# gk969/stm32-speech-recognition

Measured on AMD Instinct MI355X. Metric: utterances/sec (256-frame, 100 templates), higher is better.
Workload: dtype int32

## Files before the change

### stm32_speech_recognition_amd/csrc/k_mfcc.hip

```cpp
#include "sr_fft_dev.h"

#include <type_traits>

#ifndef SR_MEL_CHUNKED
#define SR_MEL_CHUNKED 1
#endif

namespace sr {

constexpr int kMfccWaves = 4;
constexpr int kFramesPerWave = 16, kFramesPerWaveMid = 4, kFramesPerWaveSmall = 1;
#ifndef SR_MAG_TAB_BINS
#define SR_MAG_TAB_BINS 8
#endif
constexpr int mfcc_tab_bins(int fpw) { return fpw == kFramesPerWave ? SR_MAG_TAB_BINS : 0; }
static_assert(SR_MAG_TAB_BINS == 0 || SR_MAG_TAB_BINS == 4 || SR_MAG_TAB_BINS == 8, "table bins per lane");
#ifndef SR_MFCC_PIPE
#define SR_MFCC_PIPE 1
#endif
#ifndef SR_MFCC_PIPE_PEEL
#define SR_MFCC_PIPE_PEEL 1
#endif
#ifndef SR_MFCC_PIPE_VMCNT
#define SR_MFCC_PIPE_VMCNT (SR_MFCC_PIPE_PEEL ? 3 : 0)
#endif
static_assert(SR_MFCC_PIPE_VMCNT == 0 || (SR_MFCC_PIPE_VMCNT == 3 && SR_MFCC_PIPE_PEEL), "younger loads counted by the wait");
constexpr bool mfcc_pipelined(int fpw) { return SR_MFCC_PIPE && mfcc_tab_bins(fpw) == 8; }
constexpr int kMelPad = kMel + 1;
__device__ __forceinline__ constexpr int mel_chunk_word(int j) { return 256 * ((j >> 2) & 1) + 4 * ((j >> 3) ^ (4 * ((j >> 2) & 1))) + (j & 3); }
constexpr int mfcc_wave_lds_words(int fpw) { return kXchgWords + fpw * kMelPad + 64; }

template <typename Base>
struct MfccTabArgs : Base {
    const uint16_t *mag_q;
    uint32_t mag_table_off;
};
template <typename Base>
constexpr int mfcc_feat_kind<MfccTabArgs<Base>> = mfcc_feat_kind<Base>;
template <typename Base>
static MfccTabArgs<Base> mfcc_tab_args(const Base &b, const MfccMagTab &tab)
{
    MfccTabArgs<Base> r;
    static_cast<Base &>(r) = b;
    r.mag_q = tab.mag_q;
    r.mag_table_off = tab.mag_table_off;
    return r;
}

template <int kFPW, typename Args = MfccTabArgs<MfccArgs>>
__global__ void __launch_bounds__(64 * kMfccWaves, 4) k_mfcc(const Args a)
{
    constexpr int kFeat = mfcc_feat_kind<Args>;
    constexpr uint32_t kFeatW = (kFeat == SR_FEAT_FFT || kFeat == SR_FEAT_MAG) ? kBins : kMel;
    constexpr int kWaveLdsWords = mfcc_wave_lds_words(kFPW);
    constexpr int kTabBins = mfcc_tab_bins(kFPW);
    constexpr bool kPipe = mfcc_pipelined(kFPW);
    extern __shared__ __attribute__((aligned(16))) uint32_t smem[];
    __shared__ uint32_t s_dctM[kCoef * kMelPad];
    __shared__ int s_dctS[kCoef * kMelPad];
    __shared__ u32x4 s_tw3[kTw3Row * 4], s_tw5[8 * 64];
    __shared__ u32x4 s_tm[4 * 64];
    const int lane = threadIdx.x & 63, w = __builtin_amdgcn_readfirstlane(threadIdx.x >> 6);
    uint32_t *buf = smem + w * kWaveLdsWords;
    uint32_t *xw = buf;
    uint32_t *powb = buf + kXchgWords, *moff = powb + kFPW * kMelPad;

    for (int i = threadIdx.x; i < kCoef * kMel; i += blockDim.x) {
        const int c = a.t.dct[i], o = (i / kMel) * kMelPad + i % kMel;
        s_dctM[o] = (uint32_t)(((c < 0 ? -c : c) * 262144 + 99) / 100);
        s_dctS[o] = (c > 0) - (c < 0);
    }
    __syncthreads();

    LaneTw tw;
    load_lane_tw(a.t, lane, tw);
    if (w == 0 && lane < 4) {
        const uint32_t *f = &tw.s3[0][0][0];
#pragma unroll
        for (int c = 0; c < 8; c++) s_tw3[lane * kTw3Row + c] = u32x4{f[4 * c], f[4 * c + 1], f[4 * c + 2], f[4 * c + 3]};
    }
    if (w == 1 % kMfccWaves) store_tw32(s_tw5, lane, tw.s5);
#ifndef SR_INJECT_LDS_RACE
    if (w == 2 % kMfccWaves) {
#pragma unroll
        for (int c = 0; c < 2; c++) {
            s_tm[64 * c + lane] = *(const u32x4 *)(a.t.tri_even_m + 8 * lane + 4 * c);
            s_tm[64 * (c + 2) + lane] = *(const u32x4 *)(a.t.tri_odd_m + 8 * lane + 4 * c);
        }
    }
#endif
    __syncthreads();
#ifdef SR_INJECT_LDS_RACE
    if (w == 2 % kMfccWaves) {
#if SR_INJECT_LDS_RACE >= 2
        __builtin_amdgcn_s_sleep(127);
#endif
#pragma unroll
        for (int c = 0; c < 2; c++) {
            s_tm[64 * c + lane] = *(const u32x4 *)(a.t.tri_even_m + 8 * lane + 4 * c);
            s_tm[64 * (c + 2) + lane] = *(const u32x4 *)(a.t.tri_odd_m + 8 * lane + 4 * c);
        }
    }
#endif
    int hamm_m[3];
#pragma unroll
    for (int k = 0; k < 3; k++) hamm_m[k] = (lane + 64 * k < kFrameLen) ? hamm_fused_multiplier(a.t.hamm[lane + 64 * k]) : 0;
    int f_lo = 0, p_hi = 0, p_lo = 0, x_hi = 0, x_lo = 0;
    if (lane < kMel) {
        const int h = lane;
        f_lo = (h == 0) ? 0 : (int)a.t.tri_cen[h - 1];
        const int f_hi = (h == kMel - 1) ? kBins : (int)a.t.tri_cen[h + 1];
        const int ih = f_hi - 1, il = f_lo ? f_lo - 1 : 0, half = (h & 1) ? kBins : 0;
#if SR_MEL_CHUNKED
        p_hi = half + mel_chunk_word(ih), x_hi = (ih >> 3) > 0 ? (ih >> 3) - 1 : 0;
        p_lo = half + mel_chunk_word(il), x_lo = (il >> 3) > 0 ? (il >> 3) - 1 : 0;
#else
        p_hi = half + ih, x_hi = (ih >> 3) > 0 ? (ih >> 3) - 1 : 0;
        p_lo = half + il, x_lo = (il >> 3) > 0 ? (il >> 3) - 1 : 0;
#endif
    }
    const uint64_t mag_p = (uint64_t)a.mag_q;
    const u32x4 mag_rs = {(uint32_t)mag_p, (uint32_t)(mag_p >> 32) | (2u << 16), kMagTabEntries, 0x00027000u};
    const uint32_t tw_off = 32u * (uint32_t)lane;
#if SR_MEL_CHUNKED
    const int e_base = mel_chunk_word(lane);
    constexpr int kEs = 32, kEh = 128;
    const int c0 = mel_chunk_word(8 * lane), c1 = mel_chunk_word(8 * lane + 4);
#else
    const int e_base = lane;
    constexpr int kEs = 64, kEh = 256;
    const int c0 = 8 * lane, c1 = 8 * lane + 4;
#endif

    uint32_t item = blockIdx.x;
    uint32_t nx_nfrm = 0;
    int nx_mid = 0, nx_seg0 = 0;
    if (item < a.n_items) {
        const sr_vad_rec *rec = a.vad + item / a.tiles;
        nx_nfrm = rec->frm_num;
        nx_mid = (int)rec->atap.mid_val;
        nx_seg0 = rec->seg[0];
    }
    for (; item < a.n_items; item += gridDim.x) {
        const uint32_t b = item / a.tiles, tile = item - b * a.tiles;
        const uint32_t nfrm = nx_nfrm;
        const int mid = nx_mid, seg0 = nx_seg0;
        if (item + gridDim.x < a.n_items) {
            const sr_vad_rec *rec = a.vad + (item + gridDim.x) / a.tiles;
            nx_nfrm = rec->frm_num;
            nx_mid = (int)rec->atap.mid_val;
            nx_seg0 = rec->seg[0];
        }
        const uint16_t *row = a.pcm + (uint64_t)b * a.pcm_stride;
        int16_t *out = a.mfcc + (uint64_t)b * a.max_frames * kCoef;
        const uint32_t f0 = tile * (kMfccWaves * kFPW) + w * kFPW;
        uint32_t *frow = nullptr;
        if constexpr (kFeat != 0) frow = a.feat + (uint64_t)b * a.max_frames * kFeatW;
        uint32_t nf = 0;
        if (f0 < nfrm) nf = (nfrm - f0 < (uint32_t)kFPW) ? nfrm - f0 : (uint32_t)kFPW;

        uint32_t s_pp[3] = {0, 0, 0};
        if (nf) {
            const uint16_t *x = row + seg0 + (int)kHop * (int)f0;
#pragma unroll
            for (int k = 0; k < 3; k++) {
                const int i = lane + 64 * k;
                if (i < kFrameLen) s_pp[k] = *(const u32_align2 *)(x + i - 1);
            }
        }
        if constexpr (!kPipe)
        for (uint32_t fi = 0; fi < nf; fi++) {
#pragma unroll
            for (int k = 0; k < 3; k++) {
                const int i = lane + 64 * k;
                if (i < kFrameLen) xw[i] = k == 0 ? window_sample<4>(s_pp[k], mid, hamm_m[k]) : window_sample<2>(s_pp[k], mid, hamm_m[k]);
            }
            if (fi + 1 < nf) {
                const uint16_t *x = row + seg0 + (int)kHop * (int)(f0 + fi + 1);
#pragma unroll
                for (int k = 0; k < 3; k++) {
                    const int i = lane + 64 * k;
                    if (i < kFrameLen) s_pp[k] = *(const u32_align2 *)(x + i - 1);
                }
            }
            wave_sync();
            uint32_t v[4][4], u[4][4];
            fft_front_real160(xw, lane, tw, s_tw3, v);
            fft_exchange(buf, lane, v, u);
#pragma unroll
            for (int e4 = 0; e4 < 4; e4++)
                bfly_pk<false>(u[0][e4], u[1][e4], u[2][e4], u[3][e4], tw.s4[0][0], tw.s4[0][1], tw.s4[1][0], tw.s4[1][1],
                               tw.s4[2][0], tw.s4[2][1], tw.s4[3][0], tw.s4[3][1]);
            wave_sync();
            uint32_t k5[4][4][2];
            load_tw32(s_tw5, lane, k5);
            uint32_t nn[8];
#pragma unroll
            for (int e3 = 0; e3 < 4; e3++) {
                bfly_pk<true>(u[e3][0], u[e3][1], u[e3][2], u[e3][3], k5[e3][0][0], k5[e3][0][1], k5[e3][1][0],
                              k5[e3][1][1], k5[e3][2][0], k5[e3][2][1], k5[e3][3][0], k5[e3][3][1]);
                if constexpr (kFeat == SR_FEAT_FFT) {
                    uint32_t *fr = frow + (f0 + fi) * kFeatW + lane + 64 * e3;
                    fr[0] = u[e3][0];
                    fr[256] = u[e3][1];
                }
                nn[2 * e3] = (uint32_t)sdot2z(u[e3][0], u[e3][0]);
                nn[2 * e3 + 1] = (uint32_t)sdot2z(u[e3][1], u[e3][1]);
            }
            const uint32_t nmax = max(max(max(max(nn[0], nn[1]), nn[2]), max(max(nn[3], nn[4]), nn[5])), max(nn[6], nn[7]));
#ifdef SR_TESTING
            const bool quiet = __builtin_expect(__builtin_amdgcn_ballot_w64(nmax > kMagSmallMax) == 0 && !a.mag_table_off, 1);
#else
            const bool quiet = __builtin_expect(__builtin_amdgcn_ballot_w64(nmax > kMagSmallMax) == 0, 1);
#endif
            u32x4 tw_e[2], tw_o[2];
            bool cheap = true;
            if (!quiet) {
#pragma unroll
                for (int c = 0; c < 2; c++) {
                    tw_e[c] = *(const u32x4 *)((const char *)a.t.tri_even32 + tw_off + 16 * c);
                    tw_o[c] = *(const u32x4 *)((const char *)a.t.tri_odd32 + tw_off + 16 * c);
                }
                cheap = __builtin_amdgcn_ballot_w64(nmax > a.mag_cheap_max) == 0;
            } else {
                asm volatile("" : "=v"(tw_e[0]), "=v"(tw_e[1]), "=v"(tw_o[0]), "=v"(tw_o[1]));
            }
            uint32_t *eb = buf + e_base;
            if (kTabBins > 0 && quiet) {
                uint32_t tq[8];
#pragma unroll
                for (int e3 = 0; e3 < 4; e3++) {
                    if constexpr (kTabBins == 8)
                        asm volatile("buffer_load_ushort %0, %1, %2, 0 idxen" : "=v"(tq[2 * e3]) : "v"(nn[2 * e3]), "s"(mag_rs));
                    asm volatile("buffer_load_ushort %0, %1, %2, 0 idxen" : "=v"(tq[2 * e3 + 1]) : "v"(nn[2 * e3 + 1]), "s"(mag_rs));
                }
                uint32_t q0s[4];
                if constexpr (kTabBins == 4) {
#pragma unroll
                    for (int e3 = 0; e3 < 4; e3++) q0s[e3] = cvt_u32(__builtin_amdgcn_sqrtf((float)(int)nn[2 * e3]) * 10.0f) << 2;
                }
                if constexpr (kTabBins == 8)
                    asm volatile("s_waitcnt vmcnt(0)" : "+v"(tq[0]), "+v"(tq[1]), "+v"(tq[2]), "+v"(tq[3]), "+v"(tq[4]), "+v"(tq[5]), "+v"(tq[6]), "+v"(tq[7]));
                else
                    asm volatile("s_waitcnt vmcnt(0)" : "+v"(tq[1]), "+v"(tq[3]), "+v"(tq[5]), "+v"(tq[7]));
#pragma unroll
                for (int e3 = 0; e3 < 4; e3++) {
                    uint32_t q0, q1 = tq[2 * e3 + 1];
                    if constexpr (kTabBins == 8) q0 = tq[2 * e3];
                    else q0 = q0s[e3];
                    if constexpr (kFeat == SR_FEAT_MAG) {
                        uint32_t *fr = frow + (f0 + fi) * kFeatW + lane + 64 * e3;
                        fr[0] = q0 >> 2;
                        fr[256] = q1 >> 2;
                    }
                    eb[kEs * e3] = umul24(q0, q0);
                    eb[kEs * e3 + kEh] = umul24(q1, q1);
                }
            } else if (cheap) {
#pragma unroll
                for (int e3 = 0; e3 < 4; e3++) {
                    const f32x2 m = f32x2{__builtin_amdgcn_sqrtf((float)(int)nn[2 * e3]), __builtin_amdgcn_sqrtf((float)(int)nn[2 * e3 + 1])} *
                                    f32x2{10.0f, 10.0f};
                    const uint32_t m0 = cvt_u32(m.x), m1 = cvt_u32(m.y);
                    if constexpr (kFeat == SR_FEAT_MAG) {
                        uint32_t *fr = frow + (f0 + fi) * kFeatW + lane + 64 * e3;
                        fr[0] = m0;
                        fr[256] = m1;
                    }
                    eb[kEs * e3] = umul24(m0, m0);
                    eb[kEs * e3 + kEh] = umul24(m1, m1);
                }
            } else {
#pragma unroll
                for (int e3 = 0; e3 < 4; e3++) {
                    const f32x2 m = sqrt_rn_int2(f32x2{(float)(int)nn[2 * e3], (float)(int)nn[2 * e3 + 1]}) * f32x2{10.0f, 10.0f};
                    const uint32_t m0 = cvt_u32(m.x), m1 = cvt_u32(m.y);
                    if constexpr (kFeat == SR_FEAT_MAG) {
                        uint32_t *fr = frow + (f0 + fi) * kFeatW + lane + 64 * e3;
                        fr[0] = m0;
                        fr[256] = m1;
                    }
                    eb[kEs * e3] = umul24(m0, m0);
                    eb[kEs * e3 + kEh] = umul24(m1, m1);
                }
            }
            wave_sync();
            uint32_t pe[8], po[8], xe, xo;
            {
                const uint4 q0 = *(const uint4 *)(buf + c0), q1 = *(const uint4 *)(buf + c1);
                const uint32_t e[8] = {q0.x, q0.y, q0.z, q0.w, q1.x, q1.y, q1.z, q1.w};
                uint32_t se = 0, so = 0;
                if (quiet) {
#pragma unroll
                    for (int c = 0; c < 2; c++) {
                        const u32x4 me = s_tm[64 * c + lane], mo = s_tm[64 * (c + 2) + lane];
#pragma unroll
                        for (int k = 0; k < 4; k++) {
                            const uint32_t es = kTabBins > 0 ? e[4 * c + k] : e[4 * c + k] << 4;
                            se += mel_term_fused(es, me[k]);
                            so += mel_term_fused(es, mo[k]);
                            pe[4 * c + k] = se;
                            po[4 * c + k] = so;
                        }
                    }
                } else {
#pragma unroll
                    for (int c = 0; c < 2; c++) {
#pragma unroll
                        for (int k = 0; k < 4; k++) {
                            se += e[4 * c + k] * tw_e[c][k] / 100u;
                            so += e[4 * c + k] * tw_o[c][k] / 100u;
                            pe[4 * c + k] = se;
                            po[4 * c + k] = so;
                        }
                    }
                }
                xe = wave_scan_incl(se);
                xo = wave_scan_incl(so);
            }
            *(uint4 *)(buf + c0) = make_uint4(pe[0], pe[1], pe[2], pe[3]);
            *(uint4 *)(buf + c1) = make_uint4(pe[4], pe[5], pe[6], pe[7]);
            *(uint4 *)(buf + kBins + c0) = make_uint4(po[0], po[1], po[2], po[3]);
            *(uint4 *)(buf + kBins + c1) = make_uint4(po[4], po[5], po[6], po[7]);
            buf[2 * kBins + lane] = xe;
            moff[lane] = xo;
            wave_sync();
            if (lane < kMel) {
                const uint32_t *X = (lane & 1) ? moff : buf + 2 * kBins;
                const uint32_t hi = buf[p_hi] + X[x_hi], lo = f_lo ? buf[p_lo] + X[x_lo] : 0u;
                powb[fi * kMelPad + lane] = hi - lo;
                if constexpr (kFeat == SR_FEAT_MEL) frow[(f0 + fi) * kFeatW + lane] = hi - lo;
            }
            wave_sync();
        } else {
            uint32_t mq[8] = {0, 0, 0, 0, 0, 0, 0, 0};
            bool pq = true;
            auto window = [&]() {
#pragma unroll
                for (int k = 0; k < 3; k++) {
                    const int i = lane + 64 * k;
                    if (i < kFrameLen) xw[i] = k == 0 ? window_sample<4>(s_pp[k], mid, hamm_m[k]) : window_sample<2>(s_pp[k], mid, hamm_m[k]);
                }
            };
            auto request = [&](uint32_t f) {
                const uint16_t *x = row + seg0 + (int)kHop * (int)(f0 + f);
#pragma unroll
                for (int k = 0; k < 3; k++) {
                    const int i = lane + 64 * k;
                    if (i < kFrameLen) s_pp[k] = *(const u32_align2 *)(x + i - 1);
                }
            };
            auto middle = [&](uint32_t fi, uint32_t (&v)[4][4], bool more) {
                uint32_t u[4][4];
                fft_exchange(buf, lane, v, u);
#pragma unroll
                for (int e4 = 0; e4 < 4; e4++)
                    bfly_pk<false>(u[0][e4], u[1][e4], u[2][e4], u[3][e4], tw.s4[0][0], tw.s4[0][1], tw.s4[1][0], tw.s4[1][1],
                                   tw.s4[2][0], tw.s4[2][1], tw.s4[3][0], tw.s4[3][1]);
                wave_sync();
                uint32_t k5[4][4][2];
                load_tw32(s_tw5, lane, k5);
                uint32_t nn[8];
#pragma unroll
                for (int e3 = 0; e3 < 4; e3++) {
                    bfly_pk<true>(u[e3][0], u[e3][1], u[e3][2], u[e3][3], k5[e3][0][0], k5[e3][0][1], k5[e3][1][0],
                                  k5[e3][1][1], k5[e3][2][0], k5[e3][2][1], k5[e3][3][0], k5[e3][3][1]);
                    if constexpr (kFeat == SR_FEAT_FFT) {
                        uint32_t *fr = frow + (f0 + fi) * kFeatW + lane + 64 * e3;
                        fr[0] = u[e3][0];
                        fr[256] = u[e3][1];
                    }
                    nn[2 * e3] = (uint32_t)sdot2z(u[e3][0], u[e3][0]);
                    nn[2 * e3 + 1] = (uint32_t)sdot2z(u[e3][1], u[e3][1]);
                }
                const uint32_t nmax = max(max(max(max(nn[0], nn[1]), nn[2]), max(max(nn[3], nn[4]), nn[5])), max(nn[6], nn[7]));
                if (more) {
                    wave_sync();
                    window();
                }
#ifdef SR_TESTING
                const bool quiet = __builtin_expect(__builtin_amdgcn_ballot_w64(nmax > kMagSmallMax) == 0 && !a.mag_table_off, 1);
#else
                const bool quiet = __builtin_expect(__builtin_amdgcn_ballot_w64(nmax > kMagSmallMax) == 0, 1);
#endif
                if (quiet) {
#pragma unroll
                    for (int k = 0; k < 8; k++) asm volatile("buffer_load_ushort %0, %1, %2, 0 idxen" : "=v"(mq[k]) : "v"(nn[k]), "s"(mag_rs));
                } else if (__builtin_amdgcn_ballot_w64(nmax > a.mag_cheap_max) == 0) {
#pragma unroll
                    for (int e3 = 0; e3 < 4; e3++) {
                        const f32x2 m = f32x2{__builtin_amdgcn_sqrtf((float)(int)nn[2 * e3]), __builtin_amdgcn_sqrtf((float)(int)nn[2 * e3 + 1])} *
                                        f32x2{10.0f, 10.0f};
                        mq[2 * e3] = cvt_u32(m.x);
                        mq[2 * e3 + 1] = cvt_u32(m.y);
                    }
                } else {
#pragma unroll
                    for (int e3 = 0; e3 < 4; e3++) {
                        const f32x2 m = sqrt_rn_int2(f32x2{(float)(int)nn[2 * e3], (float)(int)nn[2 * e3 + 1]}) * f32x2{10.0f, 10.0f};
                        mq[2 * e3] = cvt_u32(m.x);
                        mq[2 * e3 + 1] = cvt_u32(m.y);
                    }
                }
                pq = quiet;
                if (fi + 2 < nf) request(fi + 2);
            };
            auto back_end = [&](uint32_t r, auto young) {
                wave_sync();
                auto energies = [&]() {
                    uint32_t *eb = buf + e_base;
#pragma unroll
                    for (int e3 = 0; e3 < 4; e3++) {
                        const uint32_t q0 = mq[2 * e3], q1 = mq[2 * e3 + 1];
                        if constexpr (kFeat == SR_FEAT_MAG) {
                            uint32_t *fr = frow + (f0 + r) * kFeatW + lane + 64 * e3;
                            const uint32_t sh = pq ? 2u : 0u;
                            fr[0] = q0 >> sh;
                            fr[256] = q1 >> sh;
                        }
                        eb[kEs * e3] = umul24(q0, q0);
                        eb[kEs * e3 + kEh] = umul24(q1, q1);
                    }
                    wave_sync();
                };
                uint32_t pe[8], po[8], se = 0, so = 0;
                if (pq) {
                    if constexpr (decltype(young)::value)
                        asm volatile("s_waitcnt vmcnt(3)" : "+v"(mq[0]), "+v"(mq[1]), "+v"(mq[2]), "+v"(mq[3]), "+v"(mq[4]), "+v"(mq[5]), "+v"(mq[6]), "+v"(mq[7]));
                    else
                        asm volatile("s_waitcnt vmcnt(0)" : "+v"(mq[0]), "+v"(mq[1]), "+v"(mq[2]), "+v"(mq[3]), "+v"(mq[4]), "+v"(mq[5]), "+v"(mq[6]), "+v"(mq[7]));
                    energies();
                    const uint4 q0 = *(const uint4 *)(buf + c0), q1 = *(const uint4 *)(buf + c1);
                    const uint32_t e[8] = {q0.x, q0.y, q0.z, q0.w, q1.x, q1.y, q1.z, q1.w};
#pragma unroll
                    for (int c = 0; c < 2; c++) {
                        const u32x4 me = s_tm[64 * c + lane], mo = s_tm[64 * (c + 2) + lane];
#pragma unroll
                        for (int k = 0; k < 4; k++) {
                            se += mel_term_fused(e[4 * c + k], me[k]);
                            so += mel_term_fused(e[4 * c + k], mo[k]);
                            pe[4 * c + k] = se;
                            po[4 * c + k] = so;
                        }
                    }
                } else {
                    u32x4 tw_e[2], tw_o[2];
                    uint32_t off = tw_off;
                    asm("" : "+v"(off));
#pragma unroll
                    for (int c = 0; c < 2; c++) {
                        tw_e[c] = *(const u32x4 *)((const char *)a.t.tri_even32 + off + 16 * c);
                        tw_o[c] = *(const u32x4 *)((const char *)a.t.tri_odd32 + off + 16 * c);
                    }
                    energies();
                    const uint4 q0 = *(const uint4 *)(buf + c0), q1 = *(const uint4 *)(buf + c1);
                    const uint32_t e[8] = {q0.x, q0.y, q0.z, q0.w, q1.x, q1.y, q1.z, q1.w};
#pragma unroll
                    for (int c = 0; c < 2; c++) {
#pragma unroll
                        for (int k = 0; k < 4; k++) {
                            se += e[4 * c + k] * tw_e[c][k] / 100u;
                            so += e[4 * c + k] * tw_o[c][k] / 100u;
                            pe[4 * c + k] = se;
                            po[4 * c + k] = so;
                        }
                    }
                }
                const uint32_t xe = wave_scan_incl(se), xo = wave_scan_incl(so);
                *(uint4 *)(buf + c0) = make_uint4(pe[0], pe[1], pe[2], pe[3]);
                *(uint4 *)(buf + c1) = make_uint4(pe[4], pe[5], pe[6], pe[7]);
                *(uint4 *)(buf + kBins + c0) = make_uint4(po[0], po[1], po[2], po[3]);
                *(uint4 *)(buf + kBins + c1) = make_uint4(po[4], po[5], po[6], po[7]);
                buf[2 * kBins + lane] = xe;
                moff[lane] = xo;
                wave_sync();
                if (lane < kMel) {
                    const uint32_t *X = (lane & 1) ? moff : buf + 2 * kBins;
                    const uint32_t hi = buf[p_hi] + X[x_hi], lo = f_lo ? buf[p_lo] + X[x_lo] : 0u;
                    powb[r * kMelPad + lane] = hi - lo;
                    if constexpr (kFeat == SR_FEAT_MEL) frow[(f0 + r) * kFeatW + lane] = hi - lo;
                }
                wave_sync();
            };
            constexpr std::false_type kDrain{};
            if (nf) {
                window();
                if (nf > 1) request(1);
#if SR_MFCC_PIPE_PEEL
                constexpr std::integral_constant<bool, SR_MFCC_PIPE_VMCNT != 0> kSteady{};
                {
                    wave_sync();
                    uint32_t v[4][4];
                    fft_front_real160(xw, lane, tw, s_tw3, v);
                    middle(0, v, nf > 1);
                }
                for (uint32_t fi = 1; fi + 1 < nf; fi++) {
                    wave_sync();
                    uint32_t v[4][4];
                    fft_front_real160(xw, lane, tw, s_tw3, v);
                    back_end(fi - 1, kSteady);
                    middle(fi, v, true);
                }
                if (nf > 1) {
                    wave_sync();
                    uint32_t v[4][4];
                    fft_front_real160(xw, lane, tw, s_tw3, v);
                    back_end(nf - 2, kDrain);
                    middle(nf - 1, v, false);
                }
#else
                for (uint32_t fi = 0; fi < nf; fi++) {
                    wave_sync();
                    uint32_t v[4][4];
                    fft_front_real160(xw, lane, tw, s_tw3, v);
                    if (fi > 0) back_end(fi - 1, kDrain);
                    middle(fi, v, fi + 1 < nf);
                }
#endif
                back_end(nf - 1, kDrain);
// ... 151 lines not shown
```

### stm32_speech_recognition_amd/csrc/sr_dev.h

```cpp
#pragma once
#include <cstdlib>

#include "sr_device.h"
#include "sr_tables.h"

namespace sr {

typedef short short2v __attribute__((ext_vector_type(2)));
typedef uint32_t u32x2 __attribute__((ext_vector_type(2)));
typedef uint32_t u32x4 __attribute__((ext_vector_type(4)));

__device__ __forceinline__ int sdot2(uint32_t a, uint32_t b, int c)
{
    return __builtin_amdgcn_sdot2(__builtin_bit_cast(short2v, a), __builtin_bit_cast(short2v, b), c, false);
}
__device__ __forceinline__ int sext_lo(uint32_t w) { return (int)(short)(w & 0xFFFFu); }
__device__ __forceinline__ int sext_hi(uint32_t w) { return (int)w >> 16; }
__device__ __forceinline__ uint32_t pack16(int re, int im) { return ((uint32_t)re & 0xFFFFu) | ((uint32_t)im << 16); }

__device__ __forceinline__ int sdot2z(uint32_t a, uint32_t b)
{
    int r;
    asm("v_dot2_i32_i16 %0, %1, %2, 0" : "=v"(r) : "v"(a), "v"(b));
    return r;
}
__device__ __forceinline__ int sdot2a(uint32_t a, uint32_t b, int c)
{
    int r;
    asm("v_dot2_i32_i16 %0, %1, %2, %3" : "=v"(r) : "v"(a), "v"(b), "v"(c));
    return r;
}
__device__ __forceinline__ int preemph95(int p) { return (int)((float)p * 0.95000005f); }
__device__ __forceinline__ int neg_preemph95(int p) { return (int)((float)p * -0.95000005f); }
__device__ __forceinline__ int window_quotient(int c, int nq, int hm)
{
    int u;
    asm("v_add_lshl_u32 %0, %1, %2, %3" : "=v"(u) : "v"(c), "v"(nq), "n"(kWinShift));
    const long long P = (long long)u * (long long)hm + (long long)(unsigned long long)(uint32_t)(u >> 31);
    return (int)(P >> 32);
}
template <int SH = 2>
__device__ __forceinline__ uint32_t window_sample(uint32_t prev_cur, int mid, int hm)
{
    const int nq = neg_preemph95((int)(prev_cur & 0xFFFFu) - mid);
    const int c = (int)(prev_cur >> 16) - mid;
    int u;
    asm("v_add_lshl_u32 %0, %1, %2, %3" : "=v"(u) : "v"(c), "v"(nq), "n"(kWinShift));
    const long long P = (long long)u * (long long)hm + (long long)(unsigned long long)(uint32_t)(u >> 31);
    int r;
    asm("v_bfe_i32 %0, %1, %2, %3" : "=v"(r) : "v"((int)(P >> 32)), "n"(SH), "n"(16 - SH));
    return (uint32_t)r;
}
__device__ __forceinline__ int mul24(int a, int b) { return __mul24(a, b); }
__device__ __forceinline__ uint32_t umul24(uint32_t a, uint32_t b) { return __umul24(a, b); }
__device__ __forceinline__ int mad24(int a, int b, int c)
{
    int r;
    asm("v_mad_i32_i24 %0, %1, %2, %3" : "=v"(r) : "v"(a), "v"(b), "v"(c));
    return r;
}

__device__ __forceinline__ uint32_t mel_term_fused(uint32_t e_shl4, uint32_t m) { return __umulhi(e_shl4, m); }
__device__ __forceinline__ uint32_t mel_tri_of_multiplier(uint32_t m) { return __umulhi(m, 1600u); }

__device__ __forceinline__ float sqrt_rn_int(float f)
{
    const float y = __builtin_amdgcn_rsqf(f);
    const float s0 = f * y, h = 0.5f * y;
    const float r = __builtin_fmaf(-s0, s0, f);
    return __builtin_fmaf(r, h, s0);
}

__device__ __forceinline__ uint32_t mag10_small(float f)
{
    uint32_t r;
    const float m = __builtin_amdgcn_sqrtf(f) * 10.0f;
    asm("v_cvt_u32_f32 %0, %1" : "=v"(r) : "v"(m));
    return r;
}

__device__ __forceinline__ uint32_t cvt_u32(float x)
{
    uint32_t r;
    asm("v_cvt_u32_f32 %0, %1" : "=v"(r) : "v"(x));
    return r;
}
typedef float f32x2 __attribute__((ext_vector_type(2)));
__device__ __forceinline__ f32x2 sqrt_rn_int2(f32x2 f)
{
    const f32x2 y = {__builtin_amdgcn_rsqf(f.x), __builtin_amdgcn_rsqf(f.y)};
    const f32x2 s0 = f * y, h = f32x2{0.5f, 0.5f} * y;
    const f32x2 r = __builtin_elementwise_fma(-s0, s0, f);
    return __builtin_elementwise_fma(r, h, s0);
}
typedef uint32_t u32_align2 __attribute__((aligned(2)));
typedef uint32_t u32x2_raw __attribute__((ext_vector_type(2)));
typedef u32x2_raw u32_pair_align4 __attribute__((aligned(4)));
typedef uint32_t u32x2_align2 __attribute__((ext_vector_type(2), aligned(2)));

typedef unsigned short u16x2 __attribute__((ext_vector_type(2)));
__device__ __forceinline__ uint32_t pk_add(uint32_t a, uint32_t b)
{
    return __builtin_bit_cast(uint32_t, (u16x2)(__builtin_bit_cast(u16x2, a) + __builtin_bit_cast(u16x2, b)));
}
__device__ __forceinline__ uint32_t pk_sub(uint32_t a, uint32_t b)
{
    return __builtin_bit_cast(uint32_t, (u16x2)(__builtin_bit_cast(u16x2, a) - __builtin_bit_cast(u16x2, b)));
}
__device__ __forceinline__ uint32_t pk_ashr(uint32_t a, int n)
{
    return __builtin_bit_cast(uint32_t, (short2v)(__builtin_bit_cast(short2v, a) >> (short2v){(short)n, (short)n}));
}
__device__ __forceinline__ uint32_t pk_lshr(uint32_t a, int n)
{
    return __builtin_bit_cast(uint32_t, (u16x2)(__builtin_bit_cast(u16x2, a) >> (u16x2){(unsigned short)n, (unsigned short)n}));
}
__device__ __forceinline__ uint32_t pk_mad(uint32_t a, uint32_t c, uint32_t b)
{
    return __builtin_bit_cast(uint32_t, (u16x2)(__builtin_bit_cast(u16x2, a) * __builtin_bit_cast(u16x2, c) +
                                                __builtin_bit_cast(u16x2, b)));
}
__device__ __forceinline__ uint32_t pk_mad_swap(uint32_t a, uint32_t c, uint32_t b)
{
    uint32_t r;
    asm("v_pk_mad_u16 %0, %1, %2, %3 op_sel:[1,0,0] op_sel_hi:[0,1,1]" : "=v"(r) : "v"(a), "s"(c), "v"(b));
    return r;
}
__device__ __forceinline__ uint32_t pk_hi16(int lo_src, int hi_src)
{
    return __builtin_amdgcn_perm((uint32_t)hi_src, (uint32_t)lo_src, 0x07060302u);
}
__device__ __forceinline__ uint32_t pk_s15(int lo_src, int hi_src)
{
    uint32_t r = (uint32_t)lo_src >> 15;
    asm("v_lshrrev_b32_sdwa %0, %1, %2 dst_sel:WORD_1 dst_unused:UNUSED_PRESERVE src0_sel:DWORD src1_sel:DWORD\n\ts_nop 0"
        : "+v"(r)
        : "v"(15), "v"(hi_src));
    return r;
}

__device__ __forceinline__ void wave_sync()
{
    __builtin_amdgcn_fence(__ATOMIC_RELEASE, "wavefront");
    __builtin_amdgcn_wave_barrier();
    __builtin_amdgcn_fence(__ATOMIC_ACQUIRE, "wavefront");
}

__device__ __forceinline__ uint32_t wave_sum(uint32_t v)
{
#pragma unroll
    for (int d = 32; d >= 1; d >>= 1) v += __shfl_xor(v, d, 64);
    return v;
}
__device__ __forceinline__ uint32_t wave_min_u32(uint32_t v)
{
#pragma unroll
    for (int d = 32; d >= 1; d >>= 1) {
        uint32_t o = __shfl_xor(v, d, 64);
        v = o < v ? o : v;
    }
    return v;
}
__device__ __forceinline__ uint32_t wave_max(uint32_t v)
{
#pragma unroll
    for (int d = 32; d >= 1; d >>= 1) {
        uint32_t o = __shfl_xor(v, d, 64);
        v = o > v ? o : v;
    }
    return v;
}

template <int CTRL, int ROW_MASK>
__device__ __forceinline__ uint32_t dpp_take(uint32_t v)
{
    return (uint32_t)__builtin_amdgcn_update_dpp(0, (int)v, CTRL, ROW_MASK, 0xF, false);
}
__device__ __forceinline__ uint32_t wave_scan_incl(uint32_t v)
{
    v += dpp_take<0x111, 0xF>(v);
    v += dpp_take<0x112, 0xF>(v);
    v += dpp_take<0x114, 0xF>(v);
    v += dpp_take<0x118, 0xF>(v);
    asm("s_nop 1\n\tv_add_u32_dpp %0, %0, %0 row_bcast:15 row_mask:0xa" : "+v"(v));
    asm("s_nop 1\n\tv_add_u32_dpp %0, %0, %0 row_bcast:31 row_mask:0xc" : "+v"(v));
    return v;
}

__device__ __forceinline__ uint32_t log100_est(uint32_t n)
{
    return (uint32_t)(int)__builtin_amdgcn_fmed3f(__log2f((float)n) * 69.31471806f, 1.0f, (float)(kLogMax - 1));
}
__device__ __forceinline__ uint32_t log100_fix(uint32_t n, uint32_t m, uint32_t t0, uint32_t t1)
{
    return (uint32_t)((int)m - (int)(n < t0) + (int)(n >= t1));
}
__device__ __forceinline__ uint32_t log100_u32(uint32_t n, const uint32_t *__restrict__ thr)
{
    const uint32_t m = log100_est(n);
    return log100_fix(n, m, thr[m], thr[m + 1]);
}

}
```

### stm32_speech_recognition_amd/csrc/sr_fft_dev.h

```cpp
#pragma once
#include "sr_dev.h"

namespace sr {

__device__ __forceinline__ void cxmul(uint32_t y, uint32_t ka, uint32_t kb, int &re, int &im)
{
    re = sdot2z(y, ka);
    im = sdot2z(y, kb);
}

template <int S>
__device__ __forceinline__ void r4_combine(int &ar, int &ai, int &br, int &bi, int &cr, int &ci, int &dr, int &di)
{
    int tr = cr + dr, ti = ci + di;
    dr = cr - dr;
    di = ci - di;
    cr = tr;
    ci = ti;
    ar >>= 2;
    ai >>= 2;
    ar += br >> (2 + S);
    ai += bi >> (2 + S);
    br = ar - (br >> (1 + S));
    bi = ai - (bi >> (1 + S));
    ar += cr >> (2 + S);
    ai += ci >> (2 + S);
    cr = ar - (cr >> (1 + S));
    ci = ai - (ci >> (1 + S));
    br += di >> (2 + S);
    bi -= dr >> (2 + S);
    di = br - (di >> (1 + S));
    dr = bi + (dr >> (1 + S));
}

constexpr uint32_t kPkPlusMinus = 0xFFFF0001u;
constexpr uint32_t kPkMinusPlus = 0x0001FFFFu;

template <bool HALF, bool HAS_B, bool CD_SAME = false, bool A_SHIFTED = false>
__device__ __forceinline__ void r4_packed(uint32_t x0_in, int br, int bi, int sr, int si, int tr, int ti, uint32_t &x0,
                                          uint32_t &x1, uint32_t &x2, uint32_t &x3)
{
    const uint32_t a = A_SHIFTED ? x0_in : pk_ashr(x0_in, 2);
    uint32_t A1 = a, B1 = a;
    if (HAS_B) {
        A1 = pk_add(a, pk_hi16(br, bi));
        B1 = pk_sub(A1, pk_s15(br, bi));
    }
    const uint32_t hC = pk_hi16(sr, si);
    x0 = pk_add(A1, hC);
    x1 = CD_SAME ? pk_mad_swap(hC, kPkPlusMinus, B1) : pk_mad(pk_hi16(ti, tr), kPkPlusMinus, B1);
    if (!HALF) {
        const uint32_t pC = pk_s15(sr, si);
        x2 = pk_sub(x0, pC);
        x3 = CD_SAME ? pk_mad_swap(pC, kPkMinusPlus, x1) : pk_mad(pk_s15(ti, tr), kPkMinusPlus, x1);
    }
}

template <bool HALF>
__device__ __forceinline__ void bfly_pk(uint32_t &x0, uint32_t &x1, uint32_t &x2, uint32_t &x3, uint32_t k1a,
                                        uint32_t k1b, uint32_t k2a, uint32_t k2b, uint32_t k3a, uint32_t k3b,
                                        uint32_t k3na, uint32_t k3nb)
{
    int br, bi, cr, ci;
    cxmul(x2, k2a, k2b, cr, ci);
    cxmul(x1, k1a, k1b, br, bi);
    const int sr = sdot2a(x3, k3a, cr), si = sdot2a(x3, k3b, ci);
    const int tr = sdot2a(x3, k3na, cr), ti = sdot2a(x3, k3nb, ci);
    r4_packed<HALF, true>(x0, br, bi, sr, si, tr, ti, x0, x1, x2, x3);
}

__device__ __forceinline__ uint32_t pk_neg(uint32_t w) { return pk_sub(0u, w); }

__device__ __forceinline__ void bfly(uint32_t &x0, uint32_t &x1, uint32_t &x2, uint32_t &x3, uint32_t k1a, uint32_t k1b,
                                     uint32_t k2a, uint32_t k2b, uint32_t k3a, uint32_t k3b)
{
    bfly_pk<false>(x0, x1, x2, x3, k1a, k1b, k2a, k2b, k3a, k3b, pk_neg(k3a), pk_neg(k3b));
}

__device__ __forceinline__ int rev2(int d) { return ((d & 1) << 1) | (d >> 1); }

__device__ __forceinline__ int xaddr(int j) { return j + ((j >> 6) << 2); }
constexpr int kXchgWords = 1024 + 4 * 16;

struct LaneTw {
    uint32_t s2[2][2];
    uint32_t s3[4][4][2];
    uint32_t s4[4][2];
    uint32_t s5[4][4][2];
};

__device__ __forceinline__ void load_tw3(const DevTables &t, int base, int b, uint32_t (&k)[3][2])
{
    const int e = base + 3 * b;
    k[0][0] = t.tw_a[e + 2];
    k[0][1] = t.tw_b[e + 2];
    k[1][0] = t.tw_a[e + 1];
    k[1][1] = t.tw_b[e + 1];
    k[2][0] = t.tw_a[e + 0];
    k[2][1] = t.tw_b[e + 0];
}

__device__ __forceinline__ void load_tw4(const DevTables &t, int base, int b, uint32_t (&k)[4][2])
{
    uint32_t k3[3][2];
    load_tw3(t, base, b, k3);
#pragma unroll
    for (int e = 0; e < 3; e++) {
        k[e][0] = k3[e][0];
        k[e][1] = k3[e][1];
    }
    k[3][0] = pk_sub(0u, k3[2][0]);
    k[3][1] = pk_sub(0u, k3[2][1]);
}

__device__ __forceinline__ void load_lane_tw(const DevTables &t, int lane, LaneTw &tw)
{
    const int d0 = lane & 3;
    {
        uint32_t k[3][2];
        load_tw3(t, 0, d0, k);
        tw.s2[0][0] = k[0][0];
        tw.s2[0][1] = k[0][1];
        tw.s2[1][0] = k[1][0];
        tw.s2[1][1] = k[1][1];
    }
#pragma unroll
    for (int d1 = 0; d1 < 4; d1++) load_tw4(t, 12, d0 + 4 * d1, tw.s3[d1]);
    load_tw4(t, 60, lane, tw.s4);
#pragma unroll
    for (int d3 = 0; d3 < 4; d3++) load_tw4(t, 252, lane + 64 * d3, tw.s5[d3]);
}

__device__ __forceinline__ void store_tw32(u32x4 *lds, int lane, const uint32_t (&k)[4][4][2])
{
    const uint32_t *f = &k[0][0][0];
#pragma unroll
    for (int c = 0; c < 8; c++) lds[c * 64 + lane] = u32x4{f[4 * c], f[4 * c + 1], f[4 * c + 2], f[4 * c + 3]};
}
__device__ __forceinline__ void load_tw32(const u32x4 *lds, int lane, uint32_t (&k)[4][4][2])
{
    uint32_t *f = &k[0][0][0];
#pragma unroll
    for (int c = 0; c < 8; c++) {
        const u32x4 q = lds[c * 64 + lane];
        f[4 * c] = q.x;
        f[4 * c + 1] = q.y;
        f[4 * c + 2] = q.z;
        f[4 * c + 3] = q.w;
    }
}
constexpr int kTw3Row = 9;
__device__ __forceinline__ void load_tw32_d0(const u32x4 *lds, int d0, uint32_t (&k)[4][4][2])
{
    uint32_t *f = &k[0][0][0];
#pragma unroll
    for (int c = 0; c < 8; c++) {
        const u32x4 q = lds[d0 * kTw3Row + c];
        f[4 * c] = q.x;
        f[4 * c + 1] = q.y;
        f[4 * c + 2] = q.z;
        f[4 * c + 3] = q.w;
    }
}

__device__ __forceinline__ void fft_front_real160(const uint32_t *xw, int lane, const LaneTw &tw, const u32x4 *tw3_lds,
                                                  uint32_t (&v)[4][4])
{
    const int d3 = (lane >> 2) & 3, d4 = lane >> 4;
    const int base = rev2(d4) + 4 * rev2(d3);
    uint32_t y[10];
#pragma unroll
    for (int m = 0; m < 10; m++) y[m] = *(const uint16_t *)(xw + base + 16 * m);
#pragma unroll
    for (int m = 0; m < 4; m++) asm("" : "+v"(y[m]));
#pragma unroll
    for (int d2 = 0; d2 < 4; d2++) {
        const int r2 = ((d2 & 1) << 1) | (d2 >> 1);
        uint32_t x0 = y[r2];
        uint32_t x2 = y[4 + r2];
        uint32_t x1 = (d2 == 0) ? y[8] : (d2 == 2) ? y[9] : 0u;
        uint32_t x3 = 0u;
        int cr, ci;
        cxmul(x2, tw.s2[1][0], tw.s2[1][1], cr, ci);
        (void)x3;
        if (d2 == 0 || d2 == 2) {
            int br, bi;
            cxmul(x1, tw.s2[0][0], tw.s2[0][1], br, bi);
            r4_packed<false, true, true, true>(x0, br, bi, cr, ci, cr, ci, v[0][d2], v[1][d2], v[2][d2], v[3][d2]);
        } else {
            r4_packed<false, false, true, true>(x0, 0, 0, cr, ci, cr, ci, v[0][d2], v[1][d2], v[2][d2], v[3][d2]);
        }
    }
    uint32_t k3[4][4][2];
    load_tw32_d0(tw3_lds, lane & 3, k3);
#pragma unroll
    for (int d1 = 0; d1 < 4; d1++)
        bfly_pk<false>(v[d1][0], v[d1][1], v[d1][2], v[d1][3], k3[d1][0][0], k3[d1][0][1], k3[d1][1][0], k3[d1][1][1],
                       k3[d1][2][0], k3[d1][2][1], k3[d1][3][0], k3[d1][3][1]);
}

__device__ __forceinline__ void fft_exchange(uint32_t *buf, int lane, const uint32_t (&v)[4][4], uint32_t (&u)[4][4])
{
    const int d0 = lane & 3, d3 = (lane >> 2) & 3, d4 = lane >> 4;
    const int jw = d0 + 64 * d3 + 256 * d4;
#pragma unroll
    for (int d1 = 0; d1 < 4; d1++)
#pragma unroll
        for (int d2 = 0; d2 < 4; d2++) buf[xaddr(jw + 4 * d1 + 16 * d2)] = v[d1][d2];
    wave_sync();
#pragma unroll
    for (int e3 = 0; e3 < 4; e3++)
#pragma unroll
        for (int e4 = 0; e4 < 4; e4++) u[e3][e4] = buf[xaddr(lane + 64 * e3 + 256 * e4)];
}

__device__ __forceinline__ int bitrev8(int v) { return (int)(__brev((uint32_t)v) >> 24); }

__device__ inline void fft_full_wave(const uint32_t *__restrict__ in, uint32_t *__restrict__ out, uint32_t *buf, int lane,
                              const DevTables &t)
{
    for (int m = 0; m < 4; m++) {
        const int idx = lane + 64 * m, r = bitrev8(idx);
        const uint32_t wa = in[r], wc = in[r + 256], wb = in[r + 512], wd = in[r + 768];
        int ar = sext_lo(wa), ai = sext_hi(wa), br = sext_lo(wb), bi = sext_hi(wb);
        int cr = sext_lo(wc), ci = sext_hi(wc), dr = sext_lo(wd), di = sext_hi(wd);
        r4_combine<0>(ar, ai, br, bi, cr, ci, dr, di);
        buf[xaddr(4 * idx + 0)] = pack16(ar, ai);
        buf[xaddr(4 * idx + 1)] = pack16(br, bi);
        buf[xaddr(4 * idx + 2)] = pack16(cr, ci);
        buf[xaddr(4 * idx + 3)] = pack16(di, dr);
    }
    wave_sync();
    LaneTw tw;
    load_lane_tw(t, lane, tw);
    uint32_t k2[3][2];
    load_tw3(t, 0, lane & 3, k2);
    const int d0 = lane & 3, d3 = (lane >> 2) & 3, d4 = lane >> 4;
    uint32_t v[4][4], u[4][4];
#pragma unroll
    for (int d1 = 0; d1 < 4; d1++)
#pragma unroll
        for (int d2 = 0; d2 < 4; d2++) v[d1][d2] = buf[xaddr(d0 + 4 * d1 + 16 * d2 + 64 * d3 + 256 * d4)];
    wave_sync();
#pragma unroll
    for (int d2 = 0; d2 < 4; d2++)
        bfly(v[0][d2], v[1][d2], v[2][d2], v[3][d2], k2[0][0], k2[0][1], k2[1][0], k2[1][1], k2[2][0], k2[2][1]);
#pragma unroll
    for (int d1 = 0; d1 < 4; d1++)
        bfly(v[d1][0], v[d1][1], v[d1][2], v[d1][3], tw.s3[d1][0][0], tw.s3[d1][0][1], tw.s3[d1][1][0],
             tw.s3[d1][1][1], tw.s3[d1][2][0], tw.s3[d1][2][1]);
    fft_exchange(buf, lane, v, u);
#pragma unroll
    for (int e4 = 0; e4 < 4; e4++)
        bfly(u[0][e4], u[1][e4], u[2][e4], u[3][e4], tw.s4[0][0], tw.s4[0][1], tw.s4[1][0], tw.s4[1][1], tw.s4[2][0],
             tw.s4[2][1]);
#pragma unroll
    for (int e3 = 0; e3 < 4; e3++) {
        bfly(u[e3][0], u[e3][1], u[e3][2], u[e3][3], tw.s5[e3][0][0], tw.s5[e3][0][1], tw.s5[e3][1][0],
             tw.s5[e3][1][1], tw.s5[e3][2][0], tw.s5[e3][2][1]);
#pragma unroll
        for (int e4 = 0; e4 < 4; e4++) out[lane + 64 * e3 + 256 * e4] = u[e3][e4];
    }
}

}
```

Measured before the change: 3.262 million.

## Fold scaling into packed butterflies and pre-doubled window samples for real FFT

```diff
diff --git a/stm32_speech_recognition_amd/csrc/k_mfcc.hip b/stm32_speech_recognition_amd/csrc/k_mfcc.hip
--- a/stm32_speech_recognition_amd/csrc/k_mfcc.hip
+++ b/stm32_speech_recognition_amd/csrc/k_mfcc.hip
@@ -74,6 +74,7 @@
 
     LaneTw tw;
     load_lane_tw(a.t, lane, tw);
+    real_leg_tw(tw);
     if (w == 0 && lane < 4) {
         const uint32_t *f = &tw.s3[0][0][0];
 #pragma unroll
@@ -173,7 +174,7 @@
 #pragma unroll
             for (int k = 0; k < 3; k++) {
                 const int i = lane + 64 * k;
-                if (i < kFrameLen) xw[i] = k == 0 ? window_sample<4>(s_pp[k], mid, hamm_m[k]) : window_sample<2>(s_pp[k], mid, hamm_m[k]);
+                if (i < kFrameLen) k == 0 ? window_store<0>(xw, i, s_pp[k], mid, hamm_m[k]) : window_store<1>(xw, i, s_pp[k], mid, hamm_m[k]);
             }
             if (fi + 1 < nf) {
                 const uint16_t *x = row + seg0 + (int)kHop * (int)(f0 + fi + 1);
@@ -188,17 +189,15 @@
             fft_front_real160(xw, lane, tw, s_tw3, v);
             fft_exchange(buf, lane, v, u);
 #pragma unroll
-            for (int e4 = 0; e4 < 4; e4++)
-                bfly_pk<false>(u[0][e4], u[1][e4], u[2][e4], u[3][e4], tw.s4[0][0], tw.s4[0][1], tw.s4[1][0], tw.s4[1][1],
-                               tw.s4[2][0], tw.s4[2][1], tw.s4[3][0], tw.s4[3][1]);
+            for (int e4 = 0; e4 < 4; e4++) fft_pass4_dbl(u, e4, tw);
             wave_sync();
             uint32_t k5[4][4][2];
             load_tw32(s_tw5, lane, k5);
             uint32_t nn[8];
 #pragma unroll
             for (int e3 = 0; e3 < 4; e3++) {
-                bfly_pk<true>(u[e3][0], u[e3][1], u[e3][2], u[e3][3], k5[e3][0][0], k5[e3][0][1], k5[e3][1][0],
-                              k5[e3][1][1], k5[e3][2][0], k5[e3][2][1], k5[e3][3][0], k5[e3][3][1]);
+                bfly_pk_dbl<true, false, 0>(u[e3][0], u[e3][1], u[e3][2], u[e3][3], k5[e3][0][0], k5[e3][0][1], k5[e3][1][0],
+                                            k5[e3][1][1], k5[e3][2][0], k5[e3][2][1], k5[e3][3][0], k5[e3][3][1]);
                 if constexpr (kFeat == SR_FEAT_FFT) {
                     uint32_t *fr = frow + (f0 + fi) * kFeatW + lane + 64 * e3;
                     fr[0] = u[e3][0];
@@ -339,7 +338,7 @@
 #pragma unroll
                 for (int k = 0; k < 3; k++) {
                     const int i = lane + 64 * k;
-                    if (i < kFrameLen) xw[i] = k == 0 ? window_sample<4>(s_pp[k], mid, hamm_m[k]) : window_sample<2>(s_pp[k], mid, hamm_m[k]);
+                    if (i < kFrameLen) k == 0 ? window_store<0>(xw, i, s_pp[k], mid, hamm_m[k]) : window_store<1>(xw, i, s_pp[k], mid, hamm_m[k]);
                 }
             };
             auto request = [&](uint32_t f) {
@@ -354,17 +353,15 @@
                 uint32_t u[4][4];
                 fft_exchange(buf, lane, v, u);
 #pragma unroll
-                for (int e4 = 0; e4 < 4; e4++)
-                    bfly_pk<false>(u[0][e4], u[1][e4], u[2][e4], u[3][e4], tw.s4[0][0], tw.s4[0][1], tw.s4[1][0], tw.s4[1][1],
-                                   tw.s4[2][0], tw.s4[2][1], tw.s4[3][0], tw.s4[3][1]);
+                for (int e4 = 0; e4 < 4; e4++) fft_pass4_dbl(u, e4, tw);
                 wave_sync();
                 uint32_t k5[4][4][2];
                 load_tw32(s_tw5, lane, k5);
                 uint32_t nn[8];
 #pragma unroll
                 for (int e3 = 0; e3 < 4; e3++) {
-                    bfly_pk<true>(u[e3][0], u[e3][1], u[e3][2], u[e3][3], k5[e3][0][0], k5[e3][0][1], k5[e3][1][0],
-                                  k5[e3][1][1], k5[e3][2][0], k5[e3][2][1], k5[e3][3][0], k5[e3][3][1]);
+                    bfly_pk_dbl<true, false, 0>(u[e3][0], u[e3][1], u[e3][2], u[e3][3], k5[e3][0][0], k5[e3][0][1], k5[e3][1][0],
+                                                k5[e3][1][1], k5[e3][2][0], k5[e3][2][1], k5[e3][3][0], k5[e3][3][1]);
                     if constexpr (kFeat == SR_FEAT_FFT) {
                         uint32_t *fr = frow + (f0 + fi) * kFeatW + lane + 64 * e3;
                         fr[0] = u[e3][0];
diff --git a/stm32_speech_recognition_amd/csrc/sr_dev.h b/stm32_speech_recognition_amd/csrc/sr_dev.h
--- a/stm32_speech_recognition_amd/csrc/sr_dev.h
+++ b/stm32_speech_recognition_amd/csrc/sr_dev.h
@@ -124,6 +124,28 @@
 {
     uint32_t r;
     asm("v_pk_mad_u16 %0, %1, %2, %3 op_sel:[1,0,0] op_sel_hi:[0,1,1]" : "=v"(r) : "v"(a), "s"(c), "v"(b));
+    return r;
+}
+template <bool VC, int L1, int H1, bool SWAP = false>
+__device__ __forceinline__ uint32_t pk_mad_sel(uint32_t a, uint32_t c, uint32_t b)
+{
+    uint32_t r;
+    if constexpr (VC)
+        asm("v_pk_mad_u16 %0, %1, %2, %3 op_sel:[%4,%5,0] op_sel_hi:[%6,%7,1]" : "=v"(r) : "v"(a), "v"(c), "v"(b), "n"(SWAP ? 1 : 0), "n"(L1), "n"(SWAP ? 0 : 1), "n"(H1));
+    else
+        asm("v_pk_mad_u16 %0, %1, %2, %3 op_sel:[%4,%5,0] op_sel_hi:[%6,%7,1]" : "=v"(r) : "v"(a), "s"(c), "v"(b), "n"(SWAP ? 1 : 0), "n"(L1), "n"(SWAP ? 0 : 1), "n"(H1));
+    return r;
+}
+__device__ __forceinline__ uint32_t pk_mul_lo_lo(uint32_t a, uint32_t c)
+{
+    uint32_t r;
+    asm("v_pk_mul_lo_u16 %0, %1, %2 op_sel:[0,0] op_sel_hi:[1,0]" : "=v"(r) : "v"(a), "v"(c));
+    return r;
+}
+__device__ __forceinline__ uint32_t pk_mul_lo_dup(uint32_t a, uint32_t c)
+{
+    uint32_t r;
+    asm("v_pk_mul_lo_u16 %0, %1, %2 op_sel_hi:[0,1]" : "=v"(r) : "v"(a), "s"(c));
     return r;
 }
 __device__ __forceinline__ uint32_t pk_hi16(int lo_src, int hi_src)
diff --git a/stm32_speech_recognition_amd/csrc/sr_fft_dev.h b/stm32_speech_recognition_amd/csrc/sr_fft_dev.h
--- a/stm32_speech_recognition_amd/csrc/sr_fft_dev.h
+++ b/stm32_speech_recognition_amd/csrc/sr_fft_dev.h
@@ -1,4 +1,6 @@
 #pragma once
+#include <type_traits>
+
 #include "sr_dev.h"
 
 namespace sr {
@@ -69,6 +71,75 @@
     r4_packed<HALF, true>(x0, br, bi, sr, si, tr, ti, x0, x1, x2, x3);
 }
 
+constexpr uint32_t kPkTwo = 0xFFFE0002u;
+
+template <bool HALF, bool HAS_B, bool CD_SAME, bool DBL_CD, int OUT>
+__device__ __forceinline__ void r4_packed_dbl(uint32_t a, uint32_t mul, int br, int bi, int sr, int si, int tr, int ti,
+                                              uint32_t &x0, uint32_t &x1, uint32_t &x2, uint32_t &x3)
+{
+    auto madd = [&](uint32_t x, auto L, auto H, auto SWAP, uint32_t acc) -> uint32_t {
+        constexpr int l = decltype(L)::value, h = decltype(H)::value;
+        constexpr bool swap = decltype(SWAP)::value;
+        if constexpr (OUT == 2) return pk_mad_sel<true, l, h, swap>(x, mul, acc);
+        else if constexpr (OUT == 1) return pk_mad_sel<false, l, h, swap>(x, kPkTwo, acc);
+        else if constexpr (swap) return pk_mad_swap(x, l ? kPkMinusPlus : kPkPlusMinus, acc);
+        else if constexpr (l != h) return pk_mad(x, l ? kPkMinusPlus : kPkPlusMinus, acc);
+        else if constexpr (l) return pk_sub(acc, x);
+        else return pk_add(acc, x);
+    };
+    constexpr std::integral_constant<int, 0> P{};
+    constexpr std::integral_constant<int, 1> N{};
+    constexpr std::false_type kStraight{};
+    constexpr std::integral_constant<bool, CD_SAME> kSwapC{};
+    uint32_t A1 = a, B1 = a;
+    if (HAS_B) {
+        const uint32_t pB = pk_hi16(br, bi), hB = pk_ashr(pB, 1);
+        A1 = madd(hB, P, P, kStraight, a);
+        B1 = madd(pB, N, N, kStraight, A1);
+    }
+    uint32_t pC = 0, hC;
+    if (DBL_CD) {
+        pC = pk_hi16(sr, si);
+        hC = pk_ashr(pC, 1);
+    } else {
+        hC = pk_hi16(sr, si);
+        if (!HALF) pC = pk_s15(sr, si);
+    }
+    x0 = madd(hC, P, P, kStraight, A1);
+    uint32_t pD = 0, hD;
+    if (CD_SAME) {
+        pD = pC;
+        hD = hC;
+    } else if (DBL_CD) {
+        pD = pk_hi16(ti, tr);
+        hD = pk_ashr(pD, 1);
+    } else {
+        hD = pk_hi16(ti, tr);
+        if (!HALF) pD = pk_s15(ti, tr);
+    }
+    x1 = madd(hD, P, N, kSwapC, B1);
+    if (!HALF) {
+        x2 = madd(pC, N, N, kStraight, x0);
+        x3 = madd(pD, N, P, kSwapC, x1);
+    }
+}
+
+template <bool HALF, bool DBL_CD, int OUT>
+__device__ __forceinline__ void bfly_pk_dbl(uint32_t &x0, uint32_t &x1, uint32_t &x2, uint32_t &x3, uint32_t k1a,
+                                            uint32_t k1b, uint32_t k2a, uint32_t k2b, uint32_t k3a, uint32_t k3b,
+                                            uint32_t k3na, uint32_t k3nb, uint32_t mul = 0)
+{
+    int br, bi, cr, ci;
+    cxmul(x2, k2a, k2b, cr, ci);
+    cxmul(x1, k1a, k1b, br, bi);
+    const int sr = sdot2a(x3, k3a, cr), si = sdot2a(x3, k3b, ci);
+    const int tr = sdot2a(x3, k3na, cr), ti = sdot2a(x3, k3nb, ci);
+    uint32_t a = pk_ashr(x0, 2);
+    if (OUT == 1) a = pk_add(a, a);
+    if (OUT == 2) a = pk_mul_lo_lo(a, mul);
+    r4_packed_dbl<HALF, true, false, DBL_CD, OUT>(a, mul, br, bi, sr, si, tr, ti, x0, x1, x2, x3);
+}
+
 __device__ __forceinline__ uint32_t pk_neg(uint32_t w) { return pk_sub(0u, w); }
 
 __device__ __forceinline__ void bfly(uint32_t &x0, uint32_t &x1, uint32_t &x2, uint32_t &x3, uint32_t k1a, uint32_t k1b,
@@ -163,14 +234,36 @@
     }
 }
 
+constexpr uint32_t kPkOneTwo = 0x00020001u;
+template <int K>
+__device__ __forceinline__ void window_store(uint32_t *xw, int i, uint32_t prev_cur, int mid, int hm)
+{
+    if (K == 0) {
+        xw[i] = pk_mul_lo_dup(window_sample<4>(prev_cur, mid, hm), kPkOneTwo);
+    } else {
+        const uint32_t y = window_sample<2>(prev_cur, mid, hm);
+        xw[i] = y;
+        ((uint16_t *)(xw + i))[1] = (uint16_t)y;
+    }
+}
+__device__ __forceinline__ void real_leg_tw(LaneTw &tw)
+{
+#pragma unroll
+    for (int l = 0; l < 2; l++)
+#pragma unroll
+        for (int w = 0; w < 2; w++) tw.s2[l][w] = __builtin_amdgcn_perm(0u, tw.s2[l][w], 0x01000100u);
+}
 __device__ __forceinline__ void fft_front_real160(const uint32_t *xw, int lane, const LaneTw &tw, const u32x4 *tw3_lds,
                                                   uint32_t (&v)[4][4])
 {
     const int d3 = (lane >> 2) & 3, d4 = lane >> 4;
     const int base = rev2(d4) + 4 * rev2(d3);
     uint32_t y[10];
-#pragma unroll
-    for (int m = 0; m < 10; m++) y[m] = *(const uint16_t *)(xw + base + 16 * m);
+    y[0] = *(const uint16_t *)(xw + base);
+#pragma unroll
+    for (int m = 1; m < 4; m++) y[m] = ((const uint16_t *)(xw + base + 16 * m))[1];
+#pragma unroll
+    for (int m = 4; m < 10; m++) y[m] = xw[base + 16 * m];
 #pragma unroll
     for (int m = 0; m < 4; m++) asm("" : "+v"(y[m]));
 #pragma unroll
@@ -183,20 +276,25 @@
         int cr, ci;
         cxmul(x2, tw.s2[1][0], tw.s2[1][1], cr, ci);
         (void)x3;
-        if (d2 == 0 || d2 == 2) {
+        if (d2 == 0) {
             int br, bi;
             cxmul(x1, tw.s2[0][0], tw.s2[0][1], br, bi);
-            r4_packed<false, true, true, true>(x0, br, bi, cr, ci, cr, ci, v[0][d2], v[1][d2], v[2][d2], v[3][d2]);
+            r4_packed_dbl<false, true, true, true, 0>(x0, 0u, br, bi, cr, ci, cr, ci, v[0][d2], v[1][d2], v[2][d2], v[3][d2]);
+        } else if (d2 == 2) {
+            int br, bi;
+            cxmul(x1, tw.s2[0][0], tw.s2[0][1], br, bi);
+            r4_packed_dbl<false, true, true, true, 1>(x0, 0u, br, bi, cr, ci, cr, ci, v[0][d2], v[1][d2], v[2][d2], v[3][d2]);
         } else {
-            r4_packed<false, false, true, true>(x0, 0, 0, cr, ci, cr, ci, v[0][d2], v[1][d2], v[2][d2], v[3][d2]);
+            r4_packed_dbl<false, false, true, true, 1>(x0, 0u, 0, 0, cr, ci, cr, ci, v[0][d2], v[1][d2], v[2][d2], v[3][d2]);
         }
     }
     uint32_t k3[4][4][2];
     load_tw32_d0(tw3_lds, lane & 3, k3);
+    const uint32_t mul = d3 ? kPkTwo : kPkPlusMinus;
 #pragma unroll
     for (int d1 = 0; d1 < 4; d1++)
-        bfly_pk<false>(v[d1][0], v[d1][1], v[d1][2], v[d1][3], k3[d1][0][0], k3[d1][0][1], k3[d1][1][0], k3[d1][1][1],
-                       k3[d1][2][0], k3[d1][2][1], k3[d1][3][0], k3[d1][3][1]);
+        bfly_pk_dbl<false, true, 2>(v[d1][0], v[d1][1], v[d1][2], v[d1][3], k3[d1][0][0], k3[d1][0][1], k3[d1][1][0], k3[d1][1][1],
+                                    k3[d1][2][0], k3[d1][2][1], k3[d1][3][0], k3[d1][3][1], mul);
 }
 
 __device__ __forceinline__ void fft_exchange(uint32_t *buf, int lane, const uint32_t (&v)[4][4], uint32_t (&u)[4][4])
@@ -212,6 +310,16 @@
     for (int e3 = 0; e3 < 4; e3++)
 #pragma unroll
         for (int e4 = 0; e4 < 4; e4++) u[e3][e4] = buf[xaddr(lane + 64 * e3 + 256 * e4)];
+}
+
+__device__ __forceinline__ void fft_pass4_dbl(uint32_t (&u)[4][4], int e4, const LaneTw &tw)
+{
+    if (e4 == 1)
+        bfly_pk_dbl<false, true, 1>(u[0][e4], u[1][e4], u[2][e4], u[3][e4], tw.s4[0][0], tw.s4[0][1], tw.s4[1][0], tw.s4[1][1],
+                                    tw.s4[2][0], tw.s4[2][1], tw.s4[3][0], tw.s4[3][1]);
+    else
+        bfly_pk_dbl<false, true, 0>(u[0][e4], u[1][e4], u[2][e4], u[3][e4], tw.s4[0][0], tw.s4[0][1], tw.s4[1][0], tw.s4[1][1],
+                                    tw.s4[2][0], tw.s4[2][1], tw.s4[3][0], tw.s4[3][1]);
 }
 
 __device__ __forceinline__ int bitrev8(int v) { return (int)(__brev((uint32_t)v) >> 24); }
```

After: 3.313 million, median of 6. 1.02x the previous value.
